# stanfordnlp/mac-network

Hardware: AMD Instinct MI355X
Metric: questions/sec fwd+bwd (B=64,d=512,p=12,KB=14x14x1024) at 1/2/4/8 MI355X (higher is better)
Workload: dtype f32 (3xfp16-split emulation); 1 GPU

## Files before the change

include/macx.h:

```cpp
#ifndef MACX_H
#define MACX_H

#include <stddef.h>
#include <stdint.h>

#ifdef __cplusplus
extern "C" {
#endif

#define MACX_ABI_VERSION 5

enum {
  MACX_OK = 0,
  MACX_EINVAL = -1,
  MACX_EUNSUPPORTED = -2,
  MACX_EREJECTED = -3,
  MACX_ESMALL = -4,
  MACX_EWAIT = -5
};

enum { MACX_ACT_NON = 0, MACX_ACT_TANH = 1, MACX_ACT_SIGMOID = 2, MACX_ACT_ELU = 3, MACX_ACT_RELU = 4 };
enum { MACX_INIT_PRM = 0, MACX_INIT_ZERO = 1, MACX_INIT_Q = 2 };
enum { MACX_WRITE_MEM = 0, MACX_WRITE_INFO = 1, MACX_WRITE_SUM = 2, MACX_WRITE_BOTH = 3 };

typedef struct macx_opts {
  int32_t abi_version;
  int32_t init_ctrl, init_mem;
  int32_t control_input_unshared;
  int32_t control_input_act;
  int32_t control_feed_prev;
  int32_t control_feed_prev_att;
  int32_t control_feed_inputs;
  int32_t control_cont_act;
  int32_t read_mem_act;
  int32_t read_ctrl_act;
  int32_t write_inputs;
  int32_t write_self_att;
  int32_t write_self_att_cont;
  int32_t write_mem_act;
  int32_t write_gate;
  int32_t write_gate_shared;
  float   write_gate_bias;
  int32_t memory_variational_dropout;
  int32_t gemm_family;
  int32_t tune[16];
} macx_opts;
#define MACX_TUNE(v) ((v) + 1)
enum {
  MACX_TUNE_NATIVE_WAVES = 0,
  MACX_TUNE_PHASE_MASK = 1,
  MACX_TUNE_ROW_TILES = 2,
  MACX_TUNE_CHAIN = 4,
  MACX_TUNE_SB_DEFER = 5,
  MACX_TUNE_CHAIN_KV = 7,
  MACX_TUNE_SB_WIDE = 8,
  MACX_TUNE_WGRAD_PIPE = 10,
  MACX_TUNE_SB_CONT = 13,
  MACX_TUNE_DKB_UNI = 14,
  MACX_TUNE_PRE_FILL = 3,
  MACX_TUNE_DKB_FILL = 15
};

typedef struct macx_shapes {
  int32_t B;
  int32_t S;
  int32_t N;
  int32_t d;
  int32_t p;
  int32_t b0;
  int32_t d_logical;
} macx_shapes;

typedef struct macx_dropout {
  float keep_memory, keep_read, keep_write;
  uint32_t seed;
  const uint32_t* mask_word;
} macx_dropout;

typedef struct macx_params {
  const float* initMem;
  const float* initCtrl;
  const float* qInput_W;
  const float* qInput_b;
  const float* qInputU_W;
  const float* qInputU_b;
  const float* ctrlLogits_w;
  const float* ctrlLogits_b;
  const float* contControl_W;
  const float* contControl_b;
  const float* contControl2_W;
  const float* contControl2_b;
  const float* projX_W;
  const float* projX_b;
  const float* projY_W;
  const float* projY_b;
  const float* memKbProj_W;
  const float* memKbProj_b;
  const float* memKbProj2_W;
  const float* memKbProj2_b;
  const float* kbLogits_w;
  const float* kbLogits_b;
  const float* newMemory_W;
  const float* newMemory_b;
  const float* selfCtrl_W;
  const float* selfCtrl_b;
  const float* selfLogits_w;
  const float* selfLogits_b;
  const float* gate_W;
  const float* gate_b;
} macx_params;

typedef struct macx_param_grads {
  float* initMem; float* initCtrl;
  float* qInput_W; float* qInput_b; float* qInputU_W; float* qInputU_b;
  float* ctrlLogits_w; float* ctrlLogits_b;
  float* contControl_W; float* contControl_b; float* contControl2_W; float* contControl2_b;
  float* projX_W; float* projX_b; float* projY_W; float* projY_b;
  float* memKbProj_W; float* memKbProj_b; float* memKbProj2_W; float* memKbProj2_b;
  float* kbLogits_w; float* kbLogits_b;
  float* newMemory_W; float* newMemory_b;
  float* selfCtrl_W; float* selfCtrl_b; float* selfLogits_w; float* selfLogits_b;
  float* gate_W; float* gate_b;
} macx_param_grads;

typedef struct macx_inputs {
  const float* vecQuestions;
  const float* words;
  const int32_t* questionLengths;
  const float* knowledgeBase;
  const int32_t* kbLengths;
} macx_inputs;

typedef struct macx_input_grads {
  float* vecQuestions;
  float* words;
  float* knowledgeBase;
} macx_input_grads;

enum {
  MACX_SEG_CONTROLS = 0,
// ... 277 lines not shown
```

mac-network_amd/_lib.py:

```python
import ctypes as C
import os

import torch

from . import build as _build

ABI_VERSION = 5

MACX_OK, MACX_EINVAL, MACX_EUNSUPPORTED, MACX_EREJECTED, MACX_ESMALL, MACX_EWAIT = 0, -1, -2, -3, -4, -5
HANDOFF_BITS = {1: "a chain tile gave up waiting for its step's y", 2: "a filler workgroup gave up waiting for the previous step's write unit"}
STATUS_WORDS = 16
ACT = {"NON": 0, "TANH": 1, "SIGMOID": 2, "ELU": 3, "RELU": 4}
INIT = {"PRM": 0, "ZERO": 1, "Q": 2}
WRITE_INPUTS = {"MEM": 0, "INFO": 1, "SUM": 2, "BOTH": 3}
SEG = {"controls": 0, "memories": 1, "infos": 2, "att_question": 3, "att_kb": 4, "att_self": 5, "att_gate": 6,
       "status": 7}


class MacxOpts(C.Structure):
    _fields_ = [(n, C.c_int32) for n in (
        "abi_version", "init_ctrl", "init_mem", "control_input_unshared", "control_input_act", "control_feed_prev",
        "control_feed_prev_att", "control_feed_inputs", "control_cont_act", "read_mem_act", "read_ctrl_act",
        "write_inputs", "write_self_att", "write_self_att_cont", "write_mem_act", "write_gate", "write_gate_shared")]
    _fields_ += [("write_gate_bias", C.c_float), ("memory_variational_dropout", C.c_int32), ("gemm_family", C.c_int32),
                 ("tune", C.c_int32 * 16)]


TUNE = {"native_waves": 0, "phase_mask": 1, "row_tiles": 2, "pre_fill": 3, "chain": 4, "sb_defer": 5, "chain_kv": 7, "sb_wide": 8,
        "wgrad_pipe": 10, "sb_cont": 13, "dkb_uni": 14, "dkb_fill": 15}


def set_tune(opts, key, value):
    k = TUNE[key] if isinstance(key, str) else int(key)
    if k not in TUNE.values():
        raise KeyError("no tuning key %r (have %s)" % (key, sorted(TUNE)))
    opts.tune[k] = 0 if value is None else int(value) + 1


class MacxShapes(C.Structure):
    _fields_ = [(n, C.c_int32) for n in ("B", "S", "N", "d", "p", "b0", "d_logical")]


class MacxDropout(C.Structure):
    _fields_ = [("keep_memory", C.c_float), ("keep_read", C.c_float), ("keep_write", C.c_float), ("seed", C.c_uint32),
                ("mask_word", C.c_void_p)]


PARAM_FIELDS = (
    "initMem", "initCtrl", "qInput_W", "qInput_b", "qInputU_W", "qInputU_b", "ctrlLogits_w", "ctrlLogits_b",
    "contControl_W", "contControl_b", "contControl2_W", "contControl2_b", "projX_W", "projX_b", "projY_W", "projY_b",
    "memKbProj_W", "memKbProj_b", "memKbProj2_W", "memKbProj2_b", "kbLogits_w", "kbLogits_b", "newMemory_W",
    "newMemory_b", "selfCtrl_W", "selfCtrl_b", "selfLogits_w", "selfLogits_b", "gate_W", "gate_b")


class MacxParams(C.Structure):
    _fields_ = [(n, C.c_void_p) for n in PARAM_FIELDS]


class MacxParamGrads(C.Structure):
    _fields_ = [(n, C.c_void_p) for n in PARAM_FIELDS]


class MacxOutShapes(C.Structure):
    _fields_ = [(n, C.c_int32) for n in ("B", "d", "hidden", "answers", "b0")]


OUT_FIELDS = ("outQuestion_W", "outQuestion_b", "fc0_W", "fc0_b", "fc1_W", "fc1_b")


class MacxOutParams(C.Structure):
    _fields_ = [(n, C.c_void_p) for n in OUT_FIELDS]


class MacxOutGrads(C.Structure):
    _fields_ = [(n, C.c_void_p) for n in OUT_FIELDS]


class MacxStemShapes(C.Structure):
    _fields_ = [(n, C.c_int32) for n in ("B", "H", "W", "Cin", "Cmid", "Cout", "b0")]


STEM_FIELDS = ("kernel0", "bias0", "kernel1", "bias1")


class MacxStemParams(C.Structure):
    _fields_ = [(n, C.c_void_p) for n in STEM_FIELDS]


class MacxStemGrads(C.Structure):
    _fields_ = [(n, C.c_void_p) for n in STEM_FIELDS]


class MacxConvShapes(C.Structure):
    _fields_ = [(n, C.c_int32) for n in ("B", "H", "W", "Cin", "Cout", "k", "stride")]


class MacxEncShapes(C.Structure):
    _fields_ = [(n, C.c_int32) for n in ("B", "S", "V", "E", "h", "b0")]


ENC_FIELDS = ("emb", "fw_kernel", "fw_bias", "bw_kernel", "bw_bias")


class MacxEncParams(C.Structure):
    _fields_ = [(n, C.c_void_p) for n in ENC_FIELDS]


class MacxEncGrads(C.Structure):
    _fields_ = [(n, C.c_void_p) for n in ENC_FIELDS]


# ... 207 lines not shown
```

mac-network_amd/csrc/macx_wgrad_h2.hip.h:

```cpp
#pragma once
#include "macx_gemm_tn.hip.h"
#include "macx_h2.hip.h"

namespace macx {

__device__ __forceinline__ float sum16_h2(float v) {
  v += __shfl_xor(v, 1, 64);
  v += __shfl_xor(v, 2, 64);
  v += __shfl_xor(v, 4, 64);
  v += __shfl_xor(v, 8, 64);
  return v;
}
__device__ __forceinline__ uint32_t pk_mul_f16(uint32_t a, uint32_t b) {
  return __builtin_bit_cast(uint32_t, __builtin_bit_cast(f16x2_t, a) * __builtin_bit_cast(f16x2_t, b));
}
__device__ __forceinline__ uint32_t pk_pow2_f16(int k) {
  const float f = k < -30 ? 0.f : h2_pow2(k);
  return pk_f16(f, f);
}

struct ReadAttBwdH2P {
  int B, N, d;
  const float* att;
  const float* da;
  H2View I2;
  const float* c;
  const float* wk;
  int act;
  const uint8_t* bytes;
  float inv_keep;
  H2View dI2;
  float* dc;
  float* dwk_part;
  float* db2_part;
  float* dbk_part;
  const float* dl;
  int no_out;
};

constexpr int RABH_THREADS = 1024;
constexpr int RABH_CHUNK = 128;
__global__ __launch_bounds__(RABH_THREADS) void read_att_bwd_h2_kernel(ReadAttBwdH2P p) {
  __shared__ float s_dl[1024];
  __shared__ float s_red[RABH_THREADS / 64];
  __shared__ float s_mx[16][RABH_CHUNK];
  const int b = blockIdx.x, slab = blockIdx.y;
  const int tid = threadIdx.x, lane = tid & 63;
  const int wave = __builtin_amdgcn_readfirstlane(tid >> 6);
  constexpr int NWV = RABH_THREADS / 64;
  if (p.dl) {
    for (int n = tid; n < p.N; n += RABH_THREADS) s_dl[n] = p.dl[(size_t)b * p.N + n];
    __syncthreads();
  } else {
  float dot = 0.f;
  for (int n = tid; n < p.N; n += RABH_THREADS) dot += p.att[(size_t)b * p.N + n] * p.da[(size_t)b * p.N + n];
  dot = wave_sum(dot);
  if (lane == 0) s_red[wave] = dot;
  __syncthreads();
  dot = 0.f;
#pragma unroll
  for (int w = 0; w < NWV; ++w) dot += s_red[w];
  __syncthreads();
  float dls = 0.f;
  for (int n = tid; n < p.N; n += RABH_THREADS) {
    const float dl = p.att[(size_t)b * p.N + n] * (p.da[(size_t)b * p.N + n] - dot);
    s_dl[n] = dl;
    dls += dl;
  }
  dls = wave_sum(dls);
  if (lane == 0) s_red[wave] = dls;
  __syncthreads();
  if (tid == 0 && slab == 0) {
    float t = 0.f;
#pragma unroll
    for (int w = 0; w < NWV; ++w) t += s_red[w];
    p.dbk_part[b] = t;
  }
  }

  const int kg = slab * 16 + wave;
  const int col0 = slab * 128 + wave * 8;
  float cv[8], wv[8];
  {
    const f32x4 c0 = *reinterpret_cast<const f32x4*>(p.c + (size_t)b * p.d + col0), c1 = *reinterpret_cast<const f32x4*>(p.c + (size_t)b * p.d + col0 + 4);
    const f32x4 w0 = *reinterpret_cast<const f32x4*>(p.wk + col0), w1 = *reinterpret_cast<const f32x4*>(p.wk + col0 + 4);
// ... 61 lines not shown
          char* dst = o0 + ((size_t)kg * oRp + row) * 16;
          *reinterpret_cast<u32x4*>(dst) = hi;
          *reinterpret_cast<u32x4*>(dst + opb) = lo;
          if (wave == 0) p.dI2.exps()[row * ocb + slab] = (int8_t)ex;
        }
      }
      __syncthreads();
    }
  };
  switch (p.act) {
    case ACT_TANH: rows(std::integral_constant<int, ACT_TANH>{}); break;
    case ACT_SIGMOID: rows(std::integral_constant<int, ACT_SIGMOID>{}); break;
    case ACT_ELU: rows(std::integral_constant<int, ACT_ELU>{}); break;
    case ACT_RELU: rows(std::integral_constant<int, ACT_RELU>{}); break;
    default: rows(std::integral_constant<int, ACT_NON>{}); break;
  }
#pragma unroll
  for (int e = 0; e < 8; ++e) {
    a_dc[e] = wave_sum(a_dc[e]);
    a_dw[e] = wave_sum(a_dw[e]);
    a_db[e] = wave_sum(a_db[e]);
  }
  if (lane == 0) {
    float* dc = p.dc + (size_t)b * p.d + col0;
#pragma unroll
    for (int e = 0; e < 8; ++e) {
      dc[e] += a_dc[e];
      p.dwk_part[(size_t)b * p.d + col0 + e] = a_dw[e];
      p.db2_part[(size_t)b * p.d + col0 + e] = a_db[e];
    }
  }
}

struct TnH2P {
  int M;
  int Kd, Jd;
  int nsplit, rows_per_split;
  int R;
  const char* A; size_t a_stride; int a_mod;
  const char* G; size_t g_stride;
  const int* ecomA;
  const int* ecomG;
  int ecom_nb;
  uint16_t* ftab;
  float* part;
  int dbg;
};
__host__ __device__ inline size_t wgrad_h2_mpad(size_t M) { return (M + 63) & ~(size_t)31; }

typedef short s16x4 __attribute__((ext_vector_type(4)));
__device__ __forceinline__ u32x2 tr_read(const char* lds_addr) {
  const s16x4 v = __builtin_amdgcn_ds_read_tr16_b64_v4i16((__attribute__((address_space(3))) s16x4*)lds_addr);
  return __builtin_bit_cast(u32x2, v);
}

constexpr int WH_APL = 8 * 2 * 512;
template <int KW, int JW> constexpr int wh_stage_bytes() { return 2 * (KW + JW) * WH_APL + 256; }
template <int KW, int JW> constexpr int wh_ring() { return KW + JW == 4 ? 2 : (KW + JW == 3 ? 3 : 4); }


struct WhSlot {
  int m, kg;
  __device__ __forceinline__ int row(int row0, int nrows) const { return min(row0 + m, nrows - 1); }
};
__device__ __forceinline__ WhSlot wh_slot(int lane) { return WhSlot{(lane >> 5) * 16 + ((lane & 31) >> 1), lane & 1}; }

__device__ __forceinline__ u32x4 wh_frag(const char* tile, int lane) {
  const u32x2 lo = tr_read(tile + lane * 8), hi = tr_read(tile + 512 + lane * 8);
  return u32x4{lo[0], lo[1], hi[0], hi[1]};
}
template <int NC>
__device__ __forceinline__ void wh_load_g(const char* sg, int plane, const uint16_t* ft, int lane, u32x4 (&gf)[2][NC]) {
  ft += (lane >> 4) * 4;
  const u32x2 f0 = *reinterpret_cast<const u32x2*>(ft), f1 = *reinterpret_cast<const u32x2*>(ft + 16);
#pragma unroll
  for (int pl = 0; pl < 2; ++pl)
#pragma unroll
    for (int c = 0; c < NC; ++c) {
      u32x4 w = wh_frag(sg + pl * plane + c * 1024, lane);
      w[0] = pk_mul_f16(w[0], f0[0]); w[1] = pk_mul_f16(w[1], f0[1]);
      w[2] = pk_mul_f16(w[2], f1[0]); w[3] = pk_mul_f16(w[3], f1[1]);
      gf[pl][c] = w;
    }
}
template <int NR>
__device__ __forceinline__ void wh_load_a(const char* sa, int lane, u32x4 (&af)[NR]) {
#pragma unroll
  for (int t = 0; t < NR; ++t) af[t] = wh_frag(sa + t * 1024, lane);
}
template <int NR, int NC>
__device__ __forceinline__ void wh_mfma(const u32x4 (&af)[NR], const u32x4 (&gf)[NC], f32x4 (&acc)[NR][NC]) {
#pragma unroll
  for (int t = 0; t < NR; ++t)
#pragma unroll
    for (int c = 0; c < NC; ++c) acc[t][c] = mfma_f16(af[t], gf[c], acc[t][c]);
}
template <int NR, int NC>
__device__ __forceinline__ void wh_compute(const char* sa, int a_plane, const char* sg, int g_plane, const uint16_t* ft, int lane,
                                           f32x4 (&acc)[NR][NC]) {
  u32x4 gf[2][NC];
  wh_load_g<NC>(sg, g_plane, ft, lane, gf);
#pragma unroll
  for (int ap = 1; ap >= 0; --ap) {
    u32x4 af[NR];
    wh_load_a<NR>(sa + ap * a_plane, lane, af);
#pragma unroll
    for (int bp = 1 - ap; bp >= 0; --bp) wh_mfma<NR, NC>(af, gf[bp], acc);
  }
}
template <int NC> constexpr int wh_slab_ldw() { return 16 * NC + 4; }
template <int NT, int NR, int NC>
__device__ __forceinline__ void wh_store_slab(const f32x4 (&acc)[NR][NC], int t0, float scale, float* tw, float* out, int ld, int lane) {
  constexpr int LDW = wh_slab_ldw<NC>();
  constexpr int LPR = 4 * NC, RPI = 64 / LPR;
#pragma unroll
  for (int u = 0; u < NT; ++u)
#pragma unroll
    for (int c = 0; c < NC; ++c)
#pragma unroll
      for (int e = 0; e < 4; ++e) tw[(u * 16 + (lane >> 4) * 4 + e) * LDW + c * 16 + (lane & 15)] = acc[t0 + u][c][e] * scale;
#pragma unroll
  for (int i = 0; i < 16 * NT / RPI; ++i) {
    const int r = i * RPI + lane / LPR, c4 = (lane % LPR) * 4;
    *reinterpret_cast<f32x4*>(out + (size_t)(t0 * 16 + r) * ld + c4) = *reinterpret_cast<const f32x4*>(tw + r * LDW + c4);
  }
}

__global__ __launch_bounds__(256) void wgrad_h2_factors_kernel(TnH2P p0, TnH2P p1) {
  const TnH2P& p = blockIdx.y ? p1 : p0;
  __shared__ int sE[2][8];
  if (threadIdx.x < 16) {
    const int w = threadIdx.x >> 3, k = threadIdx.x & 7;
    sE[w][k] = h2_emin_final(w ? p.ecomG : p.ecomA, p.ecom_nb, k);
  }
  __syncthreads();
  const size_t mpad = wgrad_h2_mpad((size_t)p.M);
  const size_t m = (size_t)blockIdx.x * 256 + threadIdx.x;
  if (m >= mpad) return;
  const int acb = p.Kd >> 7, gcb = p.Jd >> 7;
  const H2View a0{const_cast<char*>(p.A), p.R, p.Kd}, g0{const_cast<char*>(p.G), p.R, p.Jd};
  if (m >= (size_t)p.M) {
    for (int i = 0; i < acb * gcb; ++i) p.ftab[(size_t)i * mpad + m] = 0;
    return;
  }
  const int ti = (int)(m / p.R), rr = (int)(m - (size_t)ti * p.R);
  const int ar = p.a_mod ? (int)(m % p.a_mod) : rr;
  const int8_t* ea = reinterpret_cast<const int8_t*>(p.A + (p.a_mod ? 0 : (size_t)ti * p.a_stride) + 2 * a0.plane_bytes()) + (size_t)ar * acb;
  const int8_t* eg = reinterpret_cast<const int8_t*>(p.G + (size_t)ti * p.g_stride + 2 * g0.plane_bytes()) + (size_t)rr * gcb;
  for (int k = 0; k < acb; ++k) {
    const int da = sE[0][k] - (int)ea[k];
    for (int j = 0; j < gcb; ++j)
      p.ftab[((size_t)k * gcb + j) * mpad + m] = (uint16_t)(pk_pow2_f16(da + sE[1][j] - (int)eg[j]) & 0xFFFFu);
  }
}

__device__ __forceinline__ void dma4b(const char* g, char* lds_wave_base) {
  const uint32_t l = __builtin_amdgcn_readfirstlane(
      (uint32_t)(uintptr_t)(__attribute__((address_space(3))) char*)lds_wave_base);
  asm volatile("s_mov_b32 m0, %1\n\ts_nop 0\n\tglobal_load_lds_dword %0, off" ::"v"(g), "s"(l) : "memory", "m0");
}

inline int wgrad_pipe_mode() { const int v = tune_get(MACX_TUNE_WGRAD_PIPE, 3); return (v >= 0 && v <= 3) ? v : 3; }

template <int KW, int JW, int PIPE = 0>
__global__ __launch_bounds__(512) void wgrad_h2_kernel(TnH2P p0, TnH2P p1) {
  const TnH2P& p = blockIdx.y ? p1 : p0;
// ... 330 lines not shown
    f32x4 y4[4];
#pragma unroll
    for (int t = 0; t < 4; ++t) y4[t] = *reinterpret_cast<const f32x4*>(ytab + (b - b_begin) * T_TILE + wr * 64 + t * 16 + (lane >> 4) * 4);
#pragma unroll
    for (int t = 0; t < 4; ++t)
#pragma unroll
      for (int e = 0; e < 4; ++e) {
        const int k = tk * T_TILE + wr * 64 + t * 16 + (lane >> 4) * 4 + e;
        const float yk = y4[t][e];
        float dyp = 0.f;
#pragma unroll
        for (int c = 0; c < 2; ++c) {
          const float sv = accS[t][c][e] * sc;
          accB[t][c][e] += sv;
          accA[t][c][e] = fmaf(yk, sv, accA[t][c][e]);
          if (DY) dyp = fmaf(w1[t][e][c], sv, dyp);
          accS[t][c][e] = 0.f;
        }
        if (DY) {
          dyp = sum16_h2(dyp);
          if ((lane & 15) == 0) p.dy_part[((size_t)(tj * 4 + wc) * p.B + b) * p.d + k] = dyp;
        }
      }
  };

#pragma unroll 1
  for (int step = 0; step < p.nsteps; ++step) {
  vX.base = p.X.base + (size_t)step * p.x_step; vG.base = p.dI1.base + (size_t)step * p.g_step;
  yS = p.y + (size_t)step * p.y_step;
  if (total > 0) {
    issue(0);
    issue(1);
    issue(2);
  }
  tables();
  if (total > 0) {
    wait_vmcnt<8>();
    __syncthreads();
    int qi = 0, qch = 0;
#pragma unroll 1
    for (int s = 0; s < total; ++s) {
      if (!(p.dbg & 2048)) issue(s + 3);
      if (!(p.dbg & 1024)) compute(s % SBH_RING, qi, qch);
      wait_vmcnt<8>();
      if (++qch == nchunk) {
        if (!(p.dbg & 512)) consume(b_begin + qi);
        qch = 0; ++qi;
      }
      __syncthreads();
    }
    wait_vmcnt<0>();
  }
  __syncthreads();
  }

  float* oa = p.dW1a_part + (size_t)group * p.d * p.d;
  float* ob = p.dW1b_part + (size_t)group * p.d * p.d;
  constexpr int LDW = 36;
  float* tw = reinterpret_cast<float*>(lds) + wave * (64 * LDW);
#pragma unroll
  for (int which = 0; which < 2; ++which) {
#pragma unroll
    for (int t = 0; t < 4; ++t)
#pragma unroll
      for (int c = 0; c < 2; ++c)
#pragma unroll
        for (int e = 0; e < 4; ++e)
          tw[(t * 16 + (lane >> 4) * 4 + e) * LDW + c * 16 + (lane & 15)] = which ? accB[t][c][e] : accA[t][c][e];
    float* o = (which ? ob : oa) + (size_t)(tk * T_TILE + wr * 64) * p.d + tj * T_TILE + wc * 32;
#pragma unroll
    for (int i = 0; i < 8; ++i) {
      const int r = i * 8 + (lane >> 3), c4 = (lane & 7) * 4;
      *reinterpret_cast<f32x4*>(o + (size_t)r * p.d + c4) = *reinterpret_cast<const f32x4*>(tw + r * LDW + c4);
    }
  }
}

constexpr int SBW_STAGE = 2 * WH_APL + 4 * WH_APL;
constexpr int SBW_RING = 3;
constexpr int SBW_MAXQ = 4;
constexpr int SBW_MAXROWS = 1024;

constexpr int SBW_TABLES = SBW_MAXROWS * 2 + SBW_MAXQ * T_TILE * 4 + 4 * SBW_MAXQ * 4;
template <bool CONT>
__global__ __launch_bounds__(512) void sb_h2w_kernel(SbH2P p) {
  extern __shared__ __attribute__((aligned(16))) float smem[];
  char* lds = reinterpret_cast<char*>(smem);
  char* tab0 = lds + SBW_RING * SBW_STAGE;
  uint16_t* ftab = reinterpret_cast<uint16_t*>(tab0);
  float* ytab = reinterpret_cast<float*>(tab0 + SBW_MAXROWS * 2);
  int* qmn = reinterpret_cast<int*>(ytab + SBW_MAXQ * T_TILE);
  float* yold = reinterpret_cast<float*>(tab0 + (CONT ? 2 : 1) * SBW_TABLES);

  const int ntk = p.d / T_TILE, ntj = p.d / (2 * T_TILE);
  const int ntile = ntk * ntj;
  const int nblk = gridDim.x;
  int v = blockIdx.x;
  if ((nblk & 7) == 0) v = (blockIdx.x & 7) * (nblk >> 3) + (blockIdx.x >> 3);
  const int group = v / ntile;
  const int tile = v % ntile;
  const int tk = tile / ntj, tj = tile % ntj;

  const int tid = threadIdx.x, lane = tid & 63;
  const int wave = __builtin_amdgcn_readfirstlane(tid >> 6);
  const int wr = wave >> 2, wc = wave & 3;
  const int gq = wc >> 1;

  const int nchunk = (p.N + 31) >> 5;
  const int b_begin = group * p.qpg;
  const int b_end = min(p.B, b_begin + p.qpg);
  const int nq = b_end - b_begin;
  const int total = nq * nchunk;
  const size_t Rp = p.X.Rp();
  const size_t xpb = p.X.plane_bytes(), gpb = p.dI1.plane_bytes();
  const int xcb = p.X.cb(), gcb = p.dI1.cb();
  H2View vX = p.X, vG = p.dI1;
  const float* yS = p.y;
  const int rows_q = nchunk * 32;

  const WhSlot sl = wh_slot(lane);
  const uint32_t lds0 = lds_addr_of(lds);
  auto issue = [&](int s_raw, int s, const char* xb, const char* gb) __attribute__((always_inline)) {
    const int qi = s / nchunk, ch = s - qi * nchunk;
    const int n = sl.row(ch * 32, p.N);
    const uint32_t voff = (uint32_t)(((size_t)sl.kg * Rp + (size_t)(b_begin + qi) * p.N + n) * 16);
    const uint32_t st = lds0 + (uint32_t)((s_raw % SBW_RING) * SBW_STAGE);
#pragma unroll
    for (int j = 0; j < 2; ++j) {
      const int u = wave * 2 + j, pl = u >> 3, ct = u & 7;
      dma16b_s(xb + pl * xpb + (size_t)(tk * 16 + 2 * ct) * Rp * 16, voff, st + pl * WH_APL + ct * 1024);
    }
#pragma unroll
    for (int j = 0; j < 4; ++j) {
      const int u = wave * 4 + j, pl = u >> 4, ct = u & 15;
      dma16b_s(gb + pl * gpb + (size_t)(tj * 32 + 2 * ct) * Rp * 16, voff, st + 2 * WH_APL + pl * 2 * WH_APL + ct * 1024);
    }
  };
  uint16_t* ftab_c = ftab;
  float* ytab_c = ytab;
  int* qmn_c = qmn;
  auto tables = [&]() __attribute__((always_inline)) {
    if (tid < 3 * SBW_MAXQ) qmn[tid] = 127;
    __syncthreads();
    for (int i0 = 0; i0 < nq * rows_q; i0 += 512) {
      const int i = i0 + tid;
      const int qi = i / rows_q, n = i - qi * rows_q;
      int ex = 127, eg0 = 127, eg1 = 127;
      if (i < nq * rows_q && n < p.N) {
        const size_t row = (size_t)(b_begin + qi) * p.N + n;
        ex = (int)vX.exps()[row * xcb + tk];
        eg0 = (int)vG.exps()[row * gcb + 2 * tj];
        eg1 = (int)vG.exps()[row * gcb + 2 * tj + 1];
      }
      const int q_lo = min(i0 + (tid & ~63), nq * rows_q - 1) / rows_q, q_hi = min(i0 + (tid | 63), nq * rows_q - 1) / rows_q;
      for (int q = q_lo; q <= q_hi; ++q) {
        int mx = qi == q ? ex : 127, mg = qi == q ? min(eg0, eg1) : 127;
#pragma unroll
        for (int o = 32; o > 0; o >>= 1) { mx = min(mx, __shfl_xor(mx, o, 64)); mg = min(mg, __shfl_xor(mg, o, 64)); }
        if (lane == 0) { atomicMin(qmn + q, mx); atomicMin(qmn + SBW_MAXQ + q, mg); }
      }
    }
    __syncthreads();
    for (int i = tid; i < 2 * nq * rows_q; i += 512) {
      const int blk = i / (nq * rows_q), r = i - blk * nq * rows_q;
      const int qi = r / rows_q, n = r - qi * rows_q;
      uint16_t f = 0;
      if (n < p.N) {
        const size_t row = (size_t)(b_begin + qi) * p.N + n;
        const int k = (min(qmn[qi], 126) - (int)vX.exps()[row * xcb + tk]) + (min(qmn[SBW_MAXQ + qi], 126) - (int)vG.exps()[row * gcb + 2 * tj + blk]);
        f = (uint16_t)(pk_pow2_f16(k) & 0xFFFFu);
      }
      ftab[blk * (SBW_MAXROWS / 2) + r] = f;
    }
    for (int i = tid; i < nq * T_TILE; i += 512)
      ytab[i] = yS[(size_t)(b_begin + (i >> 7)) * p.d + tk * T_TILE + (i & 127)];
  };

  f32x4 accT[4][4], accA[4][4];
#pragma unroll
  for (int t = 0; t < 4; ++t)
#pragma unroll
    for (int c = 0; c < 4; ++c) accT[t][c] = accA[t][c] = f32x4{0.f, 0.f, 0.f, 0.f};

  auto compute = [&](int buf, int qi, int ch) __attribute__((always_inline)) {
    const char* st = lds + buf * SBW_STAGE;
    wh_compute<4, 4>(st + (wr * 4) * 1024, WH_APL, st + 2 * WH_APL + (wc * 4) * 1024, 2 * WH_APL,
                     ftab_c + gq * (SBW_MAXROWS / 2) + qi * rows_q + ch * 32, lane, accT);
  };
  int ex_prev = 0, eg_prev = 0, ybuf = 0;
  bool pending = false;
  auto keep_y = [&](const float* ynext) __attribute__((always_inline)) {
    if (tid < T_TILE) yold[(ybuf ^ 1) * T_TILE + tid] = ynext ? ynext[tid] : 0.f;
    ybuf ^= 1;
  };
  auto fold = [&](const float* ynext, int ex_next, int eg_next) __attribute__((always_inline)) {
    const float sc = h2_unscale(ex_prev, eg_prev);
    const float mv = h2_pow2(max(min((ex_next + eg_next) - (ex_prev + eg_prev), 126), -126));
    const float* yp = yold + ybuf * T_TILE;
#pragma unroll
    for (int t = 0; t < 4; ++t) {
      const int k0 = wr * 64 + t * 16 + (lane >> 4) * 4;
      f32x4 yn = f32x4{0.f, 0.f, 0.f, 0.f};
      if (ynext) yn = *reinterpret_cast<const f32x4*>(ynext + k0);
      const f32x4 yo = *reinterpret_cast<const f32x4*>(yp + k0);
#pragma unroll
      for (int e = 0; e < 4; ++e) {
        const float dy = (yo[e] - yn[e]) * sc;
#pragma unroll
        for (int c = 0; c < 4; ++c) {
          accA[t][c][e] = fmaf(dy, accT[t][c][e], accA[t][c][e]);
          accT[t][c][e] *= mv;
        }
      }
    }
    keep_y(ynext);
    ex_prev = ex_next; eg_prev = eg_next;
  };

  if constexpr (CONT) {
    const int G = p.nsteps * total;
    auto issue_g = [&](int g_raw) __attribute__((always_inline)) {
      const int g = min(g_raw, G - 1);
      const int ist = g / total;
      issue(g_raw, g - ist * total, p.X.base + (size_t)ist * p.x_step, p.dI1.base + (size_t)ist * p.g_step);
    };
    issue_g(0);
    issue_g(1);
    tables();
    wait_vmcnt<6>();
    __syncthreads();
    const int nrows = nq * rows_q;
    const int t_q = min(tid, nrows - 1) / rows_q, t_n = min(tid, nrows - 1) - t_q * rows_q;
    const bool t_row = tid < nrows && t_n < p.N;
    const size_t t_grow = (size_t)(b_begin + t_q) * p.N + min(t_n, p.N - 1);
    const bool t_yv = tid < nq * T_TILE;
    const size_t t_yoff = (size_t)(b_begin + (t_yv ? (tid >> 7) : 0)) * p.d + tk * T_TILE + (tid & 127);
    int t_ex = 127, t_g0 = 127, t_g1 = 127;
    float t_y = 0.f;
    int step = 0, sg = 0, qi = 0, qch = 0;
#pragma unroll 1
    for (int g = 0; g < G; ++g) {
      const bool more = step + 1 < p.nsteps;
      char* nset = tab0 + ((step + 1) & 1) * SBW_TABLES;
      uint16_t* ftab_n = reinterpret_cast<uint16_t*>(nset);
      float* ytab_n = reinterpret_cast<float*>(nset + SBW_MAXROWS * 2);
      int* qmn_n = reinterpret_cast<int*>(ytab_n + SBW_MAXQ * T_TILE);
      if (more && sg == 1) {
        const H2View nX{const_cast<char*>(p.X.base) + (size_t)(step + 1) * p.x_step, p.X.R, p.X.C};
        const H2View nG{const_cast<char*>(p.dI1.base) + (size_t)(step + 1) * p.g_step, p.dI1.R, p.dI1.C};
        const int8_t* ax = nX.exps() + t_grow * xcb + tk;
        const int8_t* ag = nG.exps() + t_grow * gcb + 2 * tj;
        const float* ay = p.y + (size_t)(step + 1) * p.y_step + t_yoff;
        asm volatile("global_load_sbyte %0, %1, off" : "=v"(t_ex) : "v"(ax) : "memory");
        asm volatile("global_load_sbyte %0, %1, off" : "=v"(t_g0) : "v"(ag) : "memory");
        asm volatile("global_load_sbyte %0, %1, off offset:1" : "=v"(t_g1) : "v"(ag) : "memory");
        asm volatile("global_load_dword %0, %1, off" : "=v"(t_y) : "v"(ay) : "memory");
      }
      if (!(p.dbg & 2048)) issue_g(g + 2);
      if (qch == 0) {
        const float* yn = ytab_c + qi * T_TILE;
        const int exn = min(qmn_c[qi], 126), egn = min(qmn_c[SBW_MAXQ + qi], 126);
        if (pending) {
          if (!(p.dbg & 512)) fold(yn, exn, egn);
        } else {
          keep_y(yn);
          ex_prev = exn; eg_prev = egn;
          pending = true;
        }
      }
      if (!(p.dbg & 1024)) compute(g % SBW_RING, qi, qch);
      if (p.dbg & 2048) wait_vmcnt<0>(); else wait_vmcnt<6>();
      if (more) {
        if (sg == 0) {
          if (tid < 3 * SBW_MAXQ) qmn_n[tid] = 127;
        } else if (sg == 1) {
          asm volatile("" : "+v"(t_ex), "+v"(t_g0), "+v"(t_g1), "+v"(t_y));
          if (!t_row) { t_ex = 127; t_g0 = 127; t_g1 = 127; }
          const int q_lo = min(tid & ~63, nrows - 1) / rows_q, q_hi = min(tid | 63, nrows - 1) / rows_q;
          for (int q = q_lo; q <= q_hi; ++q) {
            int mx = t_q == q ? t_ex : 127, mg = t_q == q ? min(t_g0, t_g1) : 127;
#pragma unroll
            for (int o = 32; o > 0; o >>= 1) { mx = min(mx, __shfl_xor(mx, o, 64)); mg = min(mg, __shfl_xor(mg, o, 64)); }
            if (lane == 0) { atomicMin(qmn_n + q, mx); atomicMin(qmn_n + SBW_MAXQ + q, mg); }
          }
        } else if (sg == 2) {
          if (tid < nrows) {
            const int bx = min(qmn_n[t_q], 126), bg = min(qmn_n[SBW_MAXQ + t_q], 126);
            ftab_n[tid] = t_row ? (uint16_t)(pk_pow2_f16((bx - t_ex) + (bg - t_g0)) & 0xFFFFu) : (uint16_t)0;
            ftab_n[(SBW_MAXROWS / 2) + tid] = t_row ? (uint16_t)(pk_pow2_f16((bx - t_ex) + (bg - t_g1)) & 0xFFFFu) : (uint16_t)0;
          }
          if (t_yv) ytab_n[tid] = t_y;
        }
      }
      if (++qch == nchunk) { qch = 0; ++qi; }
      if (++sg == total) {
        sg = 0; qi = 0; ++step;
        char* cset = tab0 + (step & 1) * SBW_TABLES;
        ftab_c = reinterpret_cast<uint16_t*>(cset);
        ytab_c = reinterpret_cast<float*>(cset + SBW_MAXROWS * 2);
        qmn_c = reinterpret_cast<int*>(ytab_c + SBW_MAXQ * T_TILE);
      }
      __syncthreads();
    }
    wait_vmcnt<0>();
    __syncthreads();
  } else {
#pragma unroll 1
  for (int step = 0; step < p.nsteps; ++step) {
    vX.base = p.X.base + (size_t)step * p.x_step; vG.base = p.dI1.base + (size_t)step * p.g_step;
    yS = p.y + (size_t)step * p.y_step;
    auto issue_s = [&](int s_raw) __attribute__((always_inline)) { issue(s_raw, min(s_raw, total - 1), vX.base, vG.base); };
    if (total > 0) { issue_s(0); issue_s(1); }
    tables();
    if (total > 0) {
      wait_vmcnt<6>();
      __syncthreads();
      int qi = 0, qch = 0;
#pragma unroll 1
      for (int s = 0; s < total; ++s) {
        if (!(p.dbg & 2048)) issue_s(s + 2);
        if (qch == 0) {
          const float* yn = ytab + qi * T_TILE;
          const int exn = min(qmn[qi], 126), egn = min(qmn[SBW_MAXQ + qi], 126);
          if (pending) {
            if (!(p.dbg & 512)) fold(yn, exn, egn);
          } else {
            keep_y(yn);
            ex_prev = exn; eg_prev = egn;
            pending = true;
          }
        }
        if (!(p.dbg & 1024)) compute(s % SBW_RING, qi, qch);
        wait_vmcnt<6>();
        if (++qch == nchunk) { qch = 0; ++qi; }
        __syncthreads();
      }
      wait_vmcnt<0>();
    }
    __syncthreads();
  }
  }
  if (pending && !(p.dbg & 512)) fold(nullptr, ex_prev, eg_prev);
  const float scT = h2_unscale(ex_prev, eg_prev);

  float* tw = reinterpret_cast<float*>(lds) + wave * (64 * wh_slab_ldw<4>());
  const size_t o = (size_t)group * p.d * p.d + (size_t)(tk * T_TILE + wr * 64) * p.d + tj * 2 * T_TILE + wc * 64;
  wh_store_slab<4>(accA, 0, 1.f, tw, p.dW1a_part + o, p.d, lane);
  wh_store_slab<4>(accT, 0, scT, tw, p.dW1b_part + o, p.d, lane);
}

inline bool sb_h2_wide_ok(int B, int N, int d) { return d % 256 == 0 && B >= 1 && N >= 1 && ((N + 31) / 32) * 32 <= SBW_MAXROWS / 2; }
inline int sb_h2_wide_qpg(int B, int N, int d) {
  const int tiles = (d / 128) * (d / 256);
  int groups = 256 / tiles;
  if (groups < 1) groups = 1;
  int qpg = (B + groups - 1) / groups;
  const int rows_q = ((N + 31) / 32) * 32;
  const int cap = min(SBW_MAXQ, (SBW_MAXROWS / 2) / rows_q);
  if (qpg > cap) qpg = cap;
  return qpg < 1 ? 1 : qpg;
}
inline int sb_cont_mode() { return tune_get(MACX_TUNE_SB_CONT, 1); }
inline hipError_t sb_h2w_launch(const SbH2P& p, hipStream_t st) {
  const int nchunk = (p.N + 31) >> 5;
  if (p.qpg < 1 || p.qpg > SBW_MAXQ || p.qpg * nchunk * 32 > SBW_MAXROWS / 2 || p.d % 256 || p.dy_part || p.nsteps < 1) return hipErrorInvalidValue;
  const int ngroup = (p.B + p.qpg - 1) / p.qpg;
  const bool cont = sb_cont_mode() && p.nsteps > 1 && nchunk >= 3 && p.qpg * nchunk * 32 <= 512;
  if (cont) {
    constexpr size_t lds = (size_t)SBW_RING * SBW_STAGE + 2 * SBW_TABLES + 2 * T_TILE * 4;
    static_assert(lds <= 160 * 1024, "two table sets fit beside the ring");
    hipError_t e = lds_attr_once(reinterpret_cast<const void*>(sb_h2w_kernel<true>), lds);
    if (e != hipSuccess) return e;
    hipLaunchKernelGGL(sb_h2w_kernel<true>, dim3((p.d / 128) * (p.d / 256) * ngroup), dim3(512), lds, st, p);
    return hipGetLastError();
  }
  constexpr size_t lds = (size_t)SBW_RING * SBW_STAGE + SBW_TABLES + 2 * T_TILE * 4;
  hipError_t e = lds_attr_once(reinterpret_cast<const void*>(sb_h2w_kernel<false>), lds);
  if (e != hipSuccess) return e;
  hipLaunchKernelGGL(sb_h2w_kernel<false>, dim3((p.d / 128) * (p.d / 256) * ngroup), dim3(512), lds, st, p);
  return hipGetLastError();
}

inline hipError_t sb_h2_launch(const SbH2P& p, hipStream_t st) {
  const int nchunk = (p.N + 31) >> 5;
  if (p.qpg * nchunk * 32 > SBH_MAXROWS || p.qpg > SBH_MAXQ) return hipErrorInvalidValue;
  constexpr size_t lds = SBH_RING * SBH_STAGE + SBH_MAXROWS * 2 + SBH_MAXQ * T_TILE * 4 + SBH_MAXQ * 4 + 2 * SBH_MAXQ * 4;
  if (p.nsteps < 1 || (p.nsteps > 1 && p.dy_part)) return hipErrorInvalidValue;
  auto kern = p.dy_part ? sb_h2_kernel<true> : sb_h2_kernel<false>;
  hipError_t e = lds_attr_once(reinterpret_cast<const void*>(kern), lds);
  if (e != hipSuccess) return e;
  const int nt = p.d / T_TILE;
  const int ngroup = (p.B + p.qpg - 1) / p.qpg;
  hipLaunchKernelGGL(kern, dim3(nt * nt * ngroup), dim3(512), lds, st, p);
  return hipGetLastError();
}

}
```

Measured before the change: 17430 questions/s.

## Process two ring stages per barrier in continuous SB weight-grad kernel

Adds a variant of the continuous sb_h2w kernel that handles the shared-memory ring two stages at a time, with one barrier pair per pair of stages, and prefetches three stages deep instead of two. Fragment loads for the next stage are interleaved with MFMAs on the current stage under sched_barriers, and an odd trailing chunk is handled on its own. The aim is to cut barrier and LDS-wait stalls per chunk, at the cost of more register pressure and a more intricate handoff of next-step tables. It is selected by a new tuning key that defaults on.

After: 17570 questions/s, median of 6. Within noise of the previous version (+0.8%).

```diff
diff --git a/include/macx.h b/include/macx.h
--- a/include/macx.h
+++ b/include/macx.h
@@ -56,6 +56,7 @@
   MACX_TUNE_SB_WIDE = 8,
   MACX_TUNE_WGRAD_PIPE = 10,
   MACX_TUNE_SB_CONT = 13,
+  MACX_TUNE_SB_STAGE = 6,
   MACX_TUNE_DKB_UNI = 14,
   MACX_TUNE_PRE_FILL = 3,
   MACX_TUNE_DKB_FILL = 15
diff --git a/mac-network_amd/_lib.py b/mac-network_amd/_lib.py
--- a/mac-network_amd/_lib.py
+++ b/mac-network_amd/_lib.py
@@ -26,7 +26,7 @@
                  ("tune", C.c_int32 * 16)]
 
 
-TUNE = {"native_waves": 0, "phase_mask": 1, "row_tiles": 2, "pre_fill": 3, "chain": 4, "sb_defer": 5, "chain_kv": 7, "sb_wide": 8,
+TUNE = {"native_waves": 0, "phase_mask": 1, "row_tiles": 2, "pre_fill": 3, "chain": 4, "sb_defer": 5, "sb_stage": 6, "chain_kv": 7, "sb_wide": 8,
         "wgrad_pipe": 10, "sb_cont": 13, "dkb_uni": 14, "dkb_fill": 15}
 
 
diff --git a/mac-network_amd/csrc/macx_sb_plan.h b/mac-network_amd/csrc/macx_sb_plan.h
--- /dev/null
+++ b/mac-network_amd/csrc/macx_sb_plan.h
@@ -0,0 +1,27 @@
+#pragma once
+
+#if defined(__HIPCC__) || defined(__CUDACC__)
+#define MACX_SB_PLAN_FN __host__ __device__ constexpr
+#else
+#define MACX_SB_PLAN_FN constexpr
+#endif
+
+namespace macx {
+
+MACX_SB_PLAN_FN int sb_plan_chunks(int N) { return N <= 0 ? 0 : (N + 31) >> 5; }
+MACX_SB_PLAN_FN int sb_plan_halves(int N, int chunk) {
+  const int rows = N - 32 * chunk;
+  return rows <= 0 ? 0 : (rows <= 16 ? 1 : 2);
+}
+MACX_SB_PLAN_FN int sb_plan_stages(int N, int rows_per_stage) {
+  const int cps = rows_per_stage >> 5;
+  return (sb_plan_chunks(N) + cps - 1) / cps;
+}
+MACX_SB_PLAN_FN int sb_plan_first_chunk(int rows_per_stage, int stage) { return stage * (rows_per_stage >> 5); }
+MACX_SB_PLAN_FN int sb_plan_stage_chunks(int N, int rows_per_stage, int stage) {
+  const int cps = rows_per_stage >> 5;
+  const int left = sb_plan_chunks(N) - stage * cps;
+  return left <= 0 ? 0 : (left < cps ? left : cps);
+}
+
+}
diff --git a/mac-network_amd/csrc/macx_wgrad_h2.hip.h b/mac-network_amd/csrc/macx_wgrad_h2.hip.h
--- a/mac-network_amd/csrc/macx_wgrad_h2.hip.h
+++ b/mac-network_amd/csrc/macx_wgrad_h2.hip.h
@@ -1,6 +1,7 @@
 #pragma once
 #include "macx_gemm_tn.hip.h"
 #include "macx_h2.hip.h"
+#include "macx_sb_plan.h"
 
 namespace macx {
 
@@ -228,6 +229,18 @@
       w[2] = pk_mul_f16(w[2], f1[0]); w[3] = pk_mul_f16(w[3], f1[1]);
       gf[pl][c] = w;
     }
+}
+template <int NC>
+__device__ __forceinline__ void wh_load_g_plane(const char* sg, const uint16_t* ft, int lane, u32x4 (&gf)[NC]) {
+  ft += (lane >> 4) * 4;
+  const u32x2 f0 = *reinterpret_cast<const u32x2*>(ft), f1 = *reinterpret_cast<const u32x2*>(ft + 16);
+#pragma unroll
+  for (int c = 0; c < NC; ++c) {
+    u32x4 w = wh_frag(sg + c * 1024, lane);
+    w[0] = pk_mul_f16(w[0], f0[0]); w[1] = pk_mul_f16(w[1], f0[1]);
+    w[2] = pk_mul_f16(w[2], f1[0]); w[3] = pk_mul_f16(w[3], f1[1]);
+    gf[c] = w;
+  }
 }
 template <int NR>
 __device__ __forceinline__ void wh_load_a(const char* sa, int lane, u32x4 (&af)[NR]) {
@@ -724,7 +737,7 @@
 constexpr int SBW_MAXROWS = 1024;
 
 constexpr int SBW_TABLES = SBW_MAXROWS * 2 + SBW_MAXQ * T_TILE * 4 + 4 * SBW_MAXQ * 4;
-template <bool CONT>
+template <bool CONT, int STG = 0>
 __global__ __launch_bounds__(512) void sb_h2w_kernel(SbH2P p) {
   extern __shared__ __attribute__((aligned(16))) float smem[];
   char* lds = reinterpret_cast<char*>(smem);
@@ -859,7 +872,143 @@
     ex_prev = ex_next; eg_prev = eg_next;
   };
 
-  if constexpr (CONT) {
+  if constexpr (CONT && STG == 1) {
+    const int G = p.nsteps * total;
+    auto issue_g = [&](int g_raw) __attribute__((always_inline)) {
+      const int g = min(g_raw, G - 1);
+      const int ist = g / total;
+      issue(g_raw, g - ist * total, p.X.base + (size_t)ist * p.x_step, p.dI1.base + (size_t)ist * p.g_step);
+    };
+    issue_g(0);
+    issue_g(1);
+    issue_g(2);
+    tables();
+    wait_vmcnt<12>();
+    __syncthreads();
+    const int nrows = nq * rows_q;
+    const int t_q = min(tid, nrows - 1) / rows_q, t_n = min(tid, nrows - 1) - t_q * rows_q;
+    const bool t_row = tid < nrows && t_n < p.N;
+    const size_t t_grow = (size_t)(b_begin + t_q) * p.N + min(t_n, p.N - 1);
+    const bool t_yv = tid < nq * T_TILE;
+    const size_t t_yoff = (size_t)(b_begin + (t_yv ? (tid >> 7) : 0)) * p.d + tk * T_TILE + (tid & 127);
+    int t_ex = 127, t_g0 = 127, t_g1 = 127;
+    float t_y = 0.f;
+    const char* sa_w = lds + (wr * 4) * 1024;
+    const char* sg_w = lds + 2 * WH_APL + (wc * 4) * 1024;
+    const int n_stage = sb_plan_stages(p.N, 64);
+    const bool tail_one = sb_plan_stage_chunks(p.N, 64, n_stage - 1) == 1;
+    const int n_pair = n_stage - (tail_one ? 1 : 0);
+    int g = 0, sg = 0, slot = 0;
+#pragma unroll 1
+    for (int step = 0; step < p.nsteps; ++step) {
+      const bool more = step + 1 < p.nsteps;
+      char* nset = tab0 + ((step + 1) & 1) * SBW_TABLES;
+      uint16_t* ftab_n = reinterpret_cast<uint16_t*>(nset);
+      float* ytab_n = reinterpret_cast<float*>(nset + SBW_MAXROWS * 2);
+      int* qmn_n = reinterpret_cast<int*>(ytab_n + SBW_MAXQ * T_TILE);
+#pragma unroll 1
+    for (int qi = 0; qi < nq; ++qi) {
+      const uint16_t* ft = ftab_c + gq * (SBW_MAXROWS / 2) + qi * rows_q;
+      {
+        const float* yn = ytab_c + qi * T_TILE;
+        const int exn = min(qmn_c[qi], 126), egn = min(qmn_c[SBW_MAXQ + qi], 126);
+        if (pending) {
+          fold(yn, exn, egn);
+        } else {
+          keep_y(yn);
+          ex_prev = exn; eg_prev = egn;
+          pending = true;
+        }
+      }
+      auto first_barrier = [&]() __attribute__((always_inline)) {
+        const bool tb0 = more && sg == 0, tb2 = more && sg == 2;
+        wait_vmcnt<6>();
+        if (tb0) {
+          if (tid < 3 * SBW_MAXQ) qmn_n[tid] = 127;
+        } else if (tb2) {
+          if (tid < nrows) {
+            const int bx = min(qmn_n[t_q], 126), bg = min(qmn_n[SBW_MAXQ + t_q], 126);
+            ftab_n[tid] = t_row ? (uint16_t)(pk_pow2_f16((bx - t_ex) + (bg - t_g0)) & 0xFFFFu) : (uint16_t)0;
+            ftab_n[(SBW_MAXROWS / 2) + tid] = t_row ? (uint16_t)(pk_pow2_f16((bx - t_ex) + (bg - t_g1)) & 0xFFFFu) : (uint16_t)0;
+          }
+          if (t_yv) ytab_n[tid] = t_y;
+        }
+        __syncthreads();
+        if (tb0) {
+          const H2View nX{const_cast<char*>(p.X.base) + (size_t)(step + 1) * p.x_step, p.X.R, p.X.C};
+          const H2View nG{const_cast<char*>(p.dI1.base) + (size_t)(step + 1) * p.g_step, p.dI1.R, p.dI1.C};
+          const int8_t* ax = nX.exps() + t_grow * xcb + tk;
+          const int8_t* ag = nG.exps() + t_grow * gcb + 2 * tj;
+          const float* ay = p.y + (size_t)(step + 1) * p.y_step + t_yoff;
+          asm volatile("global_load_sbyte %0, %1, off" : "=v"(t_ex) : "v"(ax) : "memory");
+          asm volatile("global_load_sbyte %0, %1, off" : "=v"(t_g0) : "v"(ag) : "memory");
+          asm volatile("global_load_sbyte %0, %1, off offset:1" : "=v"(t_g1) : "v"(ag) : "memory");
+          asm volatile("global_load_dword %0, %1, off" : "=v"(t_y) : "v"(ay) : "memory");
+        }
+        issue_g(g + 3);
+      };
+#pragma unroll 1
+      for (int k = 0; k < n_pair; ++k) {
+        const int slot1 = slot == 2 ? 0 : slot + 1;
+        const char* sa0 = sa_w + slot * SBW_STAGE, *sg0 = sg_w + slot * SBW_STAGE;
+        const char* sa1 = sa_w + slot1 * SBW_STAGE, *sg1 = sg_w + slot1 * SBW_STAGE;
+        u32x4 gf0[2][4], gf1[2][4], af[4], af1[4];
+        wh_load_g<4>(sg0, 2 * WH_APL, ft, lane, gf0);
+        wh_load_a<4>(sa0 + WH_APL, lane, af);
+        wh_mfma<4, 4>(af, gf0[0], accT);
+        wh_load_a<4>(sa0, lane, af);
+        first_barrier();
+        wh_mfma<4, 4>(af, gf0[1], accT);
+        __builtin_amdgcn_sched_barrier(0);
+        wh_load_g_plane<4>(sg1, ft + 32, lane, gf1[0]);
+        wh_load_a<4>(sa1 + WH_APL, lane, af1);
+        wh_mfma<4, 4>(af, gf0[0], accT);
+        __builtin_amdgcn_sched_barrier(0);
+        wh_load_g_plane<4>(sg1 + 2 * WH_APL, ft + 32, lane, gf1[1]);
+        wh_load_a<4>(sa1, lane, af);
+        wh_mfma<4, 4>(af1, gf1[0], accT);
+        wait_vmcnt<6>();
+        if (more && sg == 0) {
+          asm volatile("" : "+v"(t_ex), "+v"(t_g0), "+v"(t_g1), "+v"(t_y));
+          if (!t_row) { t_ex = 127; t_g0 = 127; t_g1 = 127; }
+          const int q_lo = min(tid & ~63, nrows - 1) / rows_q, q_hi = min(tid | 63, nrows - 1) / rows_q;
+          for (int q = q_lo; q <= q_hi; ++q) {
+            int mx = t_q == q ? t_ex : 127, mg = t_q == q ? min(t_g0, t_g1) : 127;
+#pragma unroll
+            for (int o = 32; o > 0; o >>= 1) { mx = min(mx, __shfl_xor(mx, o, 64)); mg = min(mg, __shfl_xor(mg, o, 64)); }
+            if (lane == 0) { atomicMin(qmn_n + q, mx); atomicMin(qmn_n + SBW_MAXQ + q, mg); }
+          }
+        }
+        __syncthreads();
+        issue_g(g + 4);
+        wh_mfma<4, 4>(af, gf1[1], accT);
+        wh_mfma<4, 4>(af, gf1[0], accT);
+        g += 2; sg += 2; ft += 64;
+        slot = slot1 == 2 ? 0 : slot1 + 1;
+      }
+      if (tail_one) {
+        const char* sa0 = sa_w + slot * SBW_STAGE, *sg0 = sg_w + slot * SBW_STAGE;
+        u32x4 gf0[2][4], af[4];
+        wh_load_g<4>(sg0, 2 * WH_APL, ft, lane, gf0);
+        wh_load_a<4>(sa0 + WH_APL, lane, af);
+        wh_mfma<4, 4>(af, gf0[0], accT);
+        wh_load_a<4>(sa0, lane, af);
+        first_barrier();
+        wh_mfma<4, 4>(af, gf0[1], accT);
+        wh_mfma<4, 4>(af, gf0[0], accT);
+        g += 1; sg += 1;
+        slot = slot == 2 ? 0 : slot + 1;
+      }
+    }
+      sg = 0;
+      char* cset = tab0 + ((step + 1) & 1) * SBW_TABLES;
+      ftab_c = reinterpret_cast<uint16_t*>(cset);
+      ytab_c = reinterpret_cast<float*>(cset + SBW_MAXROWS * 2);
+      qmn_c = reinterpret_cast<int*>(ytab_c + SBW_MAXQ * T_TILE);
+    }
+    wait_vmcnt<0>();
+    __syncthreads();
+  } else if constexpr (CONT) {
     const int G = p.nsteps * total;
     auto issue_g = [&](int g_raw) __attribute__((always_inline)) {
       const int g = min(g_raw, G - 1);
@@ -1003,6 +1152,7 @@
   return qpg < 1 ? 1 : qpg;
 }
 inline int sb_cont_mode() { return tune_get(MACX_TUNE_SB_CONT, 1); }
+inline int sb_stage_mode() { return tune_get(MACX_TUNE_SB_STAGE, 1) ? 1 : 0; }
 inline hipError_t sb_h2w_launch(const SbH2P& p, hipStream_t st) {
   const int nchunk = (p.N + 31) >> 5;
   if (p.qpg < 1 || p.qpg > SBW_MAXQ || p.qpg * nchunk * 32 > SBW_MAXROWS / 2 || p.d % 256 || p.dy_part || p.nsteps < 1) return hipErrorInvalidValue;
@@ -1011,9 +1161,10 @@
   if (cont) {
     constexpr size_t lds = (size_t)SBW_RING * SBW_STAGE + 2 * SBW_TABLES + 2 * T_TILE * 4;
     static_assert(lds <= 160 * 1024, "two table sets fit beside the ring");
-    hipError_t e = lds_attr_once(reinterpret_cast<const void*>(sb_h2w_kernel<true>), lds);
+    auto kern = sb_stage_mode() ? sb_h2w_kernel<true, 1> : sb_h2w_kernel<true, 0>;
+    hipError_t e = lds_attr_once(reinterpret_cast<const void*>(kern), lds);
     if (e != hipSuccess) return e;
-    hipLaunchKernelGGL(sb_h2w_kernel<true>, dim3((p.d / 128) * (p.d / 256) * ngroup), dim3(512), lds, st, p);
+    hipLaunchKernelGGL(kern, dim3((p.d / 128) * (p.d / 256) * ngroup), dim3(512), lds, st, p);
     return hipGetLastError();
   }
   constexpr size_t lds = (size_t)SBW_RING * SBW_STAGE + SBW_TABLES + 2 * T_TILE * 4;
```
